# raynbowy23/RegT-GCN

Measured on AMD Instinct MI355X. Metric: training steps/sec (graph-snapshots/sec), higher is better.
Workload: dtype fp32; 1 GPU; cfg3: ONE synthetic regional graph, 100000 nodes / 1000000 edges / 8 regions, F=32, T=12, O=1, hidden=256; RegionalTemporalGCN forward+MSE+backward per snapshot, RMSprop step once per K steps (run.py semantics); gemm_arithmetic=fp32 MFMA (v_mfma_f32_32x32x2_f32), global_nodes=100000, global_edges=1000000, global_regions=8, parallelism=single GPU

## Files before the change

regt-gcn_amd/csrc/api.hip:

```cpp
#include <limits.h>
#include <stdarg.h>

#include <functional>
#include <initializer_list>
#include <map>
#include <mutex>
#include <string>
#include <unordered_map>
#include <vector>

#include "../../include/regtgcn.h"
#include <algorithm>
#include "kernels.h"

namespace regt {

static thread_local char g_err[512] = "";
void set_error(const char* fmt, ...) {
    va_list ap;
    va_start(ap, fmt);
    vsnprintf(g_err, sizeof(g_err), fmt, ap);
    va_end(ap);
}

// ... 707 lines not shown
    TRY(head_backward(d, p, gr, dpred, dhidden, hidden, L.y1, L.d1, L.dOH, L.kchunk_head, L.nchunks_head, rq, st));
    const bool split = gemm_mode() != 0 || !fp32_core_wide();
    if (split) {
        PROF("transpose_gate_w", st);
        TRY(launch_transpose3(p.gate_w[2] + C, p.gate_w[0] + C, p.gate_w[1] + C, 3, L.UT, C, C, 2L * C, st));
    }
    const bool wfr = abf && ibf && weights_frag(d) && d.regional;
    const WbPtrs wb = wb_ptrs(L.Wb, C, F, R);
    if (wfr) {
        CvtBatch cb{};
        cb.n = 3;
        for (int k = 0; k < 3; ++k) cb.t[k] = CvtTask{L.UT + (long)k * C * C, C, C, C, const_cast<float*>(wb.UT[k])};
        PROF("weights_bf16", st);
        TRY(launch_cvt_bf16_frag(cb, st));
    }
    const bool fused = wfr && !h_ext && fused_backward_ok(C) && fused_bwd_wanted();
    if (fused) {
        FusedBwdArgs a{};
        a.ZR = L.ZR; a.h = H; a.Ht = L.Ht; a.dOH = L.dOH; a.probs = L.probs;
        a.UhTf = wb.UT[0]; a.UzTf = wb.UT[1]; a.UrTf = wb.UT[2];
        a.dhp = L.dhp; a.dzr = L.dzr; a.dh = DH; a.rowdot = L.rowdot;
        a.M = M; a.T = T; a.slope = d.lrelu_slope; a.act_lrelu = d.regional ? 1 : 0; a.tile_ctr = L.tile_ctr;
        {
            PROF("fused_backward", st);
            TRY(launch_fused_backward(a, C, st));
        }
        if (gr.attention) {
            hipStream_t sa = side_fork(st);
            TRY(launch_rowdot_reduce(L.rowdot, L.dp_partial, N, T, L.cb_npb, sa));
            TRY(launch_att_bwd(L.dp_partial, L.cb_blocks, L.probs, gr.attention, T, sa));
        }
    } else {
    const bool gen = split && !ibf && !abf && gemm_dgrad1_gen_ok(M, C, N) && al16(L.Ht) && al16(L.dhp);
    if (gen) {
        GemmSegs S{};
        S.nseg = 1;
        S.seg[0] = make_seg(L.dhp, C, L.UT, nullptr, C, INT_MAX, C, true);
        S.row_div = T;
        EpiDgrad1 e{H, L.ZR, L.dOH, L.probs, L.dzr, DH, C, T};
        e.Ht = L.Ht; e.dhp = L.dhp; e.rowdot = L.rowdot; e.num_nodes = N;
        {
            PROF("dgrad_candidate", st);
            TRY(launch_gemm_dgrad1_gen(S, M, C, e, st));
        }
        if (gr.attention) {
            hipStream_t sa = side_fork(st);
            TRY(launch_rowdot_reduce(L.rowdot, L.dp_partial, N, T, L.cb_npb, sa, C / 128));
            TRY(launch_att_bwd(L.dp_partial, L.cb_blocks, L.probs, gr.attention, T, sa));
        }
    } else {
    {
        CellBwdArgs a{L.dOH, L.probs, L.ZR, H, L.Ht, L.dhp, L.dzr, L.dp_partial, N, T, C, L.cb_npb};
        a.out_bf16 = ibf; a.in_bf16 = abf;
        {
            PROF("cell_bwd", st);
            TRY(launch_cell_bwd(a, st));
        }
        if (gr.attention) TRY(launch_att_bwd(L.dp_partial, L.cb_blocks, L.probs, gr.attention, T, side_fork(st)));
    }
    {
        GemmSegs S{};
        S.nseg = 1;
        if (wfr) S.seg[0] = make_seg(L.dhp, C, wb.UT[0], nullptr, C, INT_MAX, C, true, SEG_A_BF16 | SEG_B_FRAG);
        else if (split) S.seg[0] = make_seg(L.dhp, C, L.UT, nullptr, C, INT_MAX, C, true, ibf ? SEG_A_BF16 : 0);
        else S.seg[0] = make_seg(L.dhp, C, p.gate_w[2] + C, nullptr, 2L * C, INT_MAX, C, false);
        S.row_div = T;
        EpiDgrad1 e{H, L.ZR, L.dOH, L.probs, L.dzr, DH, C, T};
        e.dzr_bf16 = ibf; e.h_bf16 = abf; e.zr_bf16 = abf; e.dh_bf16 = abf;
        PROF("dgrad_candidate", st);
        TRY(launch_gemm_dgrad1(S, M, C, e, st));
    }
    }
    if (!tcol) {
        GemmSegs S{};
        S.nseg = 2;
        if (wfr) {
            S.seg[0] = make_seg(byte_off(L.dzr, 2L * C), 2L * C, wb.UT[2], nullptr, C, INT_MAX, C, true, SEG_A_BF16 | SEG_B_FRAG);
            S.seg[1] = make_seg(L.dzr, 2L * C, wb.UT[1], nullptr, C, INT_MAX, C, true, SEG_A_BF16 | SEG_B_FRAG);
        } else if (split) {
            const int fl = ibf ? SEG_A_BF16 : 0;
            S.seg[0] = make_seg(byte_off(L.dzr, (ibf ? 2L : 4L) * C), 2L * C, L.UT + 2L * C * C, nullptr, C, INT_MAX, C, true, fl);
            S.seg[1] = make_seg(L.dzr, 2L * C, L.UT + (long)C * C, nullptr, C, INT_MAX, C, true, fl);
        } else {
            S.seg[0] = make_seg(L.dzr, 2L * C, p.gate_w[0] + C, nullptr, 2L * C, INT_MAX, C, false);
            S.seg[1] = make_seg(L.dzr + C, 2L * C, p.gate_w[1] + C, nullptr, 2L * C, INT_MAX, C, false);
        }
        S.row_div = T;
        EpiDgrad2 e{DH, H, C, d.regional ? ACT_LRELU : ACT_NONE, d.lrelu_slope};
        e.h_bf16 = abf; e.dh_bf16 = abf;
        PROF("dgrad_gates", st);
        TRY(launch_gemm_dgrad2(S, M, C, e, st));
    }
    }
    const int pairs_opt = option(OPT_WGRAD_PAIRS);
    const bool pairs = (pairs_opt == 2 ? wgrad_ring_active() : pairs_opt == 1) && ibf && qbf && abf && xbf && !h_ext && !tcol && C % 128 == 0 && F % 8 == 0;
    if (pairs) {
        int kc = L.kchunk, nc = L.nchunks;
        wgrad_ring_chunking(C, C + F, M, &kc, &nc);
        WgradArgs a{L.dhp, C, C, L.q, C, C + F, 0, M, kc, nullptr, nc, nullptr, 1};
        a.p_bf16 = 1; a.q_bf16 = 1; a.Q2 = L.AX; a.ldq2 = F; a.nin_split = C;
        TRY(rq.take((long)nc * wgrad_slab_stride(a), &a.slab));
        {
            PROF("wgrad_UhGh", st);
            TRY(launch_wgrad(a, st));
        }
        WgradReduceArgs r{};
        r.slab = a.slab; r.nchunks = nc; r.slab_stride = wgrad_slab_stride(a); r.slab_ld = C + F; r.ngroups = 1;
        r.elem_offset = 0; r.Nout = C; r.Nin = C; r.out = gr.gate_w[2] + C; r.ldo = 2L * C;
        r.colsum_out = L.dch; r.colsum_offset = (long)C * (C + F); r.ncolsum = C;
        TRY(rq.push(r));
        WgradReduceArgs g{};
        g.slab = a.slab; g.nchunks = nc; g.slab_stride = wgrad_slab_stride(a); g.slab_ld = C + F; g.ngroups = 1;
        g.elem_offset = C; g.Nout = C; g.Nin = F; g.out = L.dGh; g.ldo = F;
        TRY(rq.push(g));
    } else {
    {
        int kc = L.kchunk, nc = L.nchunks;
        if (!ibf && !qbf) wgrad_wide_chunking(C, C, M, &kc, &nc);
        TRY(wgrad_full(rq, "wgrad_Uh", L.dhp, C, C, L.q, C, C, 0, M, kc, nc, gr.gate_w[2] + C, 2L * C, L.dch, st, ibf, qbf));
    }
    {
        int kc = L.kchunk_s, nc = L.nchunks_s;
        if (!ibf && !xbf && F <= 32) wgrad_skinny_chunking(C, M, &kc, &nc);
        TRY(wgrad_full(rq, "wgrad_Gh", L.dhp, C, C, L.AX, F, F, 0, M, kc, nc, L.dGh, F, nullptr, st, ibf, xbf));
// ... 765 lines not shown
```

regt-gcn_amd/csrc/gemm.hip:

```cpp
#include "kernels.h"
#include "gemm_fast.h"
#include "gemm_split.h"
#include "gemm_small.h"

namespace regt {

#ifdef REGT_WG_TRACE
__device__ long g_wg_trace[4 * WG_TRACE_MAX];
__device__ long g_wg_marks[8 * WG_TRACE_MAX];
#define WG_TRACE_T(name) const long name = wall_clock64()
#define WG_TRACE_END(N, ta, tb)                                                                                              \
    if (threadIdx.x == 0 && WG_TILE_ID < WG_TRACE_MAX && (N) == REGT_WG_TRACE_N) {                                            \
        long* q_ = g_wg_trace + 4L * WG_TILE_ID;                                                                              \
        q_[0] = ta; q_[1] = tb; q_[2] = wall_clock64();                                                                       \
        q_[3] = ((long)__builtin_amdgcn_s_getreg((31 << 11) | 4)) | ((long)__builtin_amdgcn_s_getreg((31 << 11) | 20) << 32); \
    }
#else
#define WG_TRACE_T(name)
#define WG_TRACE_END(N, ta, tb)
#endif

__device__ __forceinline__ float fast_sigmoid(float x) { return __builtin_amdgcn_rcpf(1.0f + __expf(-x)); }
__device__ __forceinline__ float fast_tanh(float x) { return 1.0f - 2.0f * __builtin_amdgcn_rcpf(1.0f + __expf(2.0f * x)); }
__device__ __forceinline__ float4 ld4(const float* p) { return *reinterpret_cast<const float4*>(p); }
// ... 188 lines not shown
        if (V & 1) buf_st4_bf16(t.dzr, t.vdzr + i * t.sdzr, 0, REGT_V4(F_));
        else buf_st4(t.dzr, t.vdzr + i * t.sdzr, 0, REGT_V4(F_));
#undef F_
#define F_(k) cb_dh(v.k, a.R.k, a.p, a.d.k, a.Z.k)
        buf_st4(t.dh, t.vc + i * t.sc, 0, REGT_V4(F_));
#undef F_
    }
};
struct EpiDgrad1GenF {
    EpiDgrad1 e;
    int parts;
    static constexpr int ROUND_ROWS = 8;
    __device__ __forceinline__ static float half_wave_sum(float s) {
#define REGT_DPP_ADD(ctrl, rmask) s += __builtin_bit_cast(float, __builtin_amdgcn_update_dpp(0, __builtin_bit_cast(int, s), ctrl, rmask, 0xF, true))
        REGT_DPP_ADD(0xB1, 0xF);
        REGT_DPP_ADD(0x4E, 0xF);
        REGT_DPP_ADD(0x141, 0xF);
        REGT_DPP_ADD(0x140, 0xF);
        REGT_DPP_ADD(0x142, 0xA);
#undef REGT_DPP_ADD
        return s;
    }
    static constexpr int SUM_LANE = 31;
    static constexpr int EPI_AUX_BYTES = 192;
    struct Aux { float4 h, Z, R, d, t; float p; };
    __device__ __forceinline__ Aux load(long m, int c) const {
        const long node = m / e.T;
        Aux a;
        a.p = e.probs[(int)(m - node * e.T)];
        a.h = ld4(e.h + m * e.C + c);
        a.Z = ld4(e.ZR + m * (2L * e.C) + c);
        a.R = ld4(e.ZR + m * (2L * e.C) + e.C + c);
        a.d = ld4(e.dOH + node * e.C + c);
        a.t = ld4(e.Ht + m * e.C + c);
        return a;
    }
#define REGT_GEN_DOT(a) ((a.d.x * (a.Z.x * a.h.x + (1.0f - a.Z.x) * a.t.x) + a.d.y * (a.Z.y * a.h.y + (1.0f - a.Z.y) * a.t.y)) + \
                         (a.d.z * (a.Z.z * a.h.z + (1.0f - a.Z.z) * a.t.z) + a.d.w * (a.Z.w * a.h.w + (1.0f - a.Z.w) * a.t.w)))
    __device__ __forceinline__ void apply(long m, int c, float4 v, const Aux& a) const {
#define F_(k) cb_drp(v.k, a.h.k, a.R.k)
        st4(e.dzr + m * (2L * e.C) + e.C + c, REGT_V4(F_));
#undef F_
#define F_(k) cb_dh(v.k, a.R.k, a.p, a.d.k, a.Z.k)
        st4(e.dh + m * e.C + c, REGT_V4(F_));
#undef F_
#define F_(k) cb_dzp(__fmul_rn(a.p, a.d.k), a.h.k, a.t.k, a.Z.k)
        st4(e.dzr + m * (2L * e.C) + c, REGT_V4(F_));
#undef F_
        const float s = half_wave_sum(REGT_GEN_DOT(a));
        if ((threadIdx.x & 31) == SUM_LANE) e.rowdot[m * parts + c / GBN] = s;
    }
    static constexpr int NVAR = 1;
    static constexpr bool HAS_ROWTAB = true;
    struct Col {};
    struct Tile { __amdgpu_buffer_rsrc_t h, zr, d, dzr, dh, t, rd; int vc, vzr, sc, szr, vd, vrd, srd, rstep; const EpiRowEnt* rt; };
    __device__ __forceinline__ int variant(int) const { return 0; }
    __device__ __forceinline__ EpiRowEnt vrow(long m) const {
        const long node = m / e.T;
        return EpiRowEnt{(int)(node * e.C * 4), e.probs[(int)(m - node * e.T)]};
    }
    template <int V> __device__ __forceinline__ Col vcol(int) const { return Col{}; }
    template <int V> __device__ __forceinline__ Tile vtile(const EpiGeom& g) const {
        Tile t;
        t.h = buf_srd(e.h + g.m0 * e.C + g.n0);
        t.t = buf_srd(e.Ht + g.m0 * e.C + g.n0);
        t.dh = buf_srd(e.dh + g.m0 * e.C + g.n0);
        t.zr = buf_srd(e.ZR + g.m0 * (2L * e.C) + g.n0);
        t.d = buf_srd(e.dOH + g.n0);
        t.dzr = buf_srd(e.dzr + g.m0 * (2L * e.C) + g.n0);
        t.rd = buf_srd(e.rowdot + g.m0 * parts + g.n0 / GBN);
        t.vc = (g.rr * e.C + g.c) * 4;
        t.sc = g.step * e.C * 4;
        t.vzr = 2 * t.vc - g.c * 4;
        t.szr = 2 * t.sc;
        t.vd = g.c * 4;
        t.vrd = g.rr * parts * 4;
        t.srd = g.step * parts * 4;
        t.rt = g.rowtab + g.rr;
        t.rstep = g.step;
        return t;
    }
    struct VAux { float4 h, Z, R, d, t; float p; };
    template <int V> __device__ __forceinline__ VAux vload(const Tile& t, int i) const {
        const EpiRowEnt re = t.rt[i * t.rstep];
        VAux a;
        a.p = re.p;
        a.h = buf_ld4(t.h, t.vc, i * t.sc);
        a.Z = buf_ld4(t.zr, t.vzr, i * t.szr);
        a.R = buf_ld4(t.zr, t.vzr, i * t.szr + e.C * 4);
        a.d = buf_ld4(t.d, t.vd + re.off, 0);
        a.t = buf_ld4(t.t, t.vc, i * t.sc);
        return a;
    }
    template <int V> __device__ __forceinline__ void vapply(const Tile& t, int i, float4 v, const Col&, const VAux& a) const {
#define F_(k) cb_drp(v.k, a.h.k, a.R.k)
        buf_st4(t.dzr, t.vzr + i * t.szr + e.C * 4, 0, REGT_V4(F_));
#undef F_
#define F_(k) cb_dh(v.k, a.R.k, a.p, a.d.k, a.Z.k)
        buf_st4(t.dh, t.vc + i * t.sc, 0, REGT_V4(F_));
#undef F_
#define F_(k) cb_dzp(__fmul_rn(a.p, a.d.k), a.h.k, a.t.k, a.Z.k)
        buf_st4(t.dzr, t.vzr + i * t.szr, 0, REGT_V4(F_));
#undef F_
        const float s = half_wave_sum(REGT_GEN_DOT(a));
        if ((threadIdx.x & 31) == SUM_LANE) __builtin_amdgcn_raw_buffer_store_b32(__float_as_uint(s), t.rd, t.vrd + i * t.srd, 0, 0);
    }
#undef REGT_GEN_DOT
};
struct EpiDgrad2F {
    EpiDgrad2 e;
    __device__ __forceinline__ void operator()(long m, int c, float v) const {
        long i = m * e.C + c;
        float d = e.dh[i] + v;
        if (e.act == ACT_LRELU) d = e.h[i] > 0.f ? d : d * e.slope;
        e.dh[i] = d;
    }
    static constexpr int ROUND_ROWS = 16;
    struct Aux { float4 d, h; };
    __device__ __forceinline__ Aux load(long m, int c) const {
        Aux a;
        a.d = ld4(e.dh + m * e.C + c);
        a.h = e.act == ACT_LRELU ? ld4(e.h + m * e.C + c) : make_float4(1, 1, 1, 1);
        return a;
    }
    __device__ __forceinline__ void apply(long m, int c, float4 v, const Aux& a) const {
#define F_(k) ((a.d.k + v.k) * (a.h.k > 0.f ? 1.0f : e.slope))
        st4(e.dh + m * e.C + c, REGT_V4(F_));
#undef F_
    }
    static constexpr int NVAR = 2;
    static constexpr bool HAS_ROWTAB = false;
    struct Col {};
    struct VAux { float4 d, h; };
    struct Tile { __amdgpu_buffer_rsrc_t dh, h; int v, s; };
    __device__ __forceinline__ int variant(int) const { return e.act == ACT_LRELU ? 1 : 0; }
    template <int V> __device__ __forceinline__ Col vcol(int) const { return Col{}; }
    template <int V> __device__ __forceinline__ Tile vtile(const EpiGeom& g) const {
        Tile t;
        t.dh = buf_srd(e.dh + g.m0 * e.C + g.n0);
        if (V & 1) t.h = buf_srd(e.h + g.m0 * e.C + g.n0);
        t.v = (g.rr * e.C + g.c) * 4;
        t.s = g.step * e.C * 4;
        return t;
    }
    template <int V> __device__ __forceinline__ VAux vload(const Tile& t, int i) const {
        VAux a;
        a.d = buf_ld4(t.dh, t.v, i * t.s);
        if (V & 1) a.h = buf_ld4(t.h, t.v, i * t.s);
        return a;
    }
    template <int V> __device__ __forceinline__ void vapply(const Tile& t, int i, float4 v, const Col&, const VAux& a) const {
#define F_(k) ((a.d.k + v.k) * ((V & 1) ? (a.h.k > 0.f ? 1.0f : e.slope) : 1.0f))
        buf_st4(t.dh, t.v + i * t.s, 0, REGT_V4(F_));
#undef F_
    }
};
struct EpiMaskAddF {
    EpiMaskAdd e;
    __device__ __forceinline__ void operator()(long m, int c, float v) const {
        float o = e.mask[m * e.ldm + c] > 0.f ? v : 0.f;
        if (e.add) o += e.add[m * e.ldadd + c];
        e.out[m * e.ldo + c] = o;
    }
    static constexpr int ROUND_ROWS = 16;
    struct Aux { float4 mk, ad; };
    __device__ __forceinline__ Aux load(long m, int c) const {
        Aux a;
        a.mk = ld4(e.mask + m * e.ldm + c);
        a.ad = e.add ? ld4(e.add + m * e.ldadd + c) : make_float4(0, 0, 0, 0);
        return a;
    }
    __device__ __forceinline__ void apply(long m, int c, float4 v, const Aux& a) const {
#define F_(k) ((a.mk.k > 0.f ? v.k : 0.f) + a.ad.k)
        st4(e.out + m * e.ldo + c, REGT_V4(F_));
#undef F_
    }
    static constexpr int NVAR = 2;
    static constexpr bool HAS_ROWTAB = false;
    struct Col {};
    struct VAux { float4 mk, ad; };
    struct Tile { __amdgpu_buffer_rsrc_t out, mask, add; int vo, vm, va, so, sm, sa; };
    __device__ __forceinline__ int variant(int) const {
        return (e.ldo >= (1L << 22) || e.ldm >= (1L << 22) || (e.add && e.ldadd >= (1L << 22))) ? -1 : (e.add ? 1 : 0);
    }
    template <int V> __device__ __forceinline__ Col vcol(int) const { return Col{}; }
    template <int V> __device__ __forceinline__ Tile vtile(const EpiGeom& g) const {
        Tile t;
// ... 350 lines not shown
#pragma unroll
    for (int i = 0; i < 2; ++i)
#pragma unroll
        for (int j = 0; j < 2; ++j)
#pragma unroll
            for (int r = 0; r < 16; ++r) acc[i][j][r] = 0.f;
    WG_TRACE_T(t_a);
    if (uni) core.run_uniform(acc, relu_a != 0);
    else core.run(acc, relu_a != 0);
    WG_TRACE_T(t_b);
    core.for_each_vec_halves(acc, epi);
    WG_TRACE_END(N, t_a, t_b);
}

template <int NP>
__global__ __launch_bounds__(256, 2) void gemm_dgrad1_gen_kernel(GemmSegs S, long M, int N, EpiDgrad1GenF epi) {
    extern __shared__ __attribute__((aligned(16))) float lds[];
    const int tiles_n = (N + GBN - 1) / GBN;
    const int bid = xcd_remap(blockIdx.x, gridDim.x);
    const long m0 = (long)(bid / tiles_n) * GBM;
    const int n0 = (bid % tiles_n) * GBN;
    RowMap rm{m0, 1, (int)((M - m0) < GBM ? (M - m0) : GBM)};
    SplitCore<false, NP> core(S, rm, n0, N, lds, true);
    core.fill_rowtab(epi);
    f32x16 acc[2][2];
#pragma unroll
    for (int i = 0; i < 2; ++i)
#pragma unroll
        for (int j = 0; j < 2; ++j)
#pragma unroll
            for (int r = 0; r < 16; ++r) acc[i][j][r] = 0.f;
    const typename SplitCore<false, NP>::AGen g{epi.e.ZR, epi.e.Ht, epi.e.dOH, epi.e.dhp, epi.e.C, (unsigned)epi.e.num_nodes * (unsigned)epi.e.C * 4u};
    core.run_u_gen(acc, g);
    core.for_each_vec_halves(acc, epi);
}

template <class EpiF8, bool REGION>
__global__ __launch_bounds__(256, 3) void gemm_flat_split8_kernel(GemmSegs S, long M, int N, EpiF8 epi, int uniform) {
    extern __shared__ __attribute__((aligned(16))) float lds[];
    const int tiles_n = (N + GBN - 1) / GBN;
    const int bid = xcd_remap(blockIdx.x, gridDim.x);
    const long m0 = (long)(bid / tiles_n) * GBM;
    const int n0 = (bid % tiles_n) * GBN;
    RowMap rm{m0, 1, (int)((M - m0) < GBM ? (M - m0) : GBM)};
    SplitCore<REGION, 1> core(S, rm, n0, N, lds, true);
    core.fill_rowtab(epi);
    const bool uni = uniform != 0;
    if (!uni) core.plan();
    f32x16 acc[2][2];
#pragma unroll
    for (int i = 0; i < 2; ++i)
#pragma unroll
        for (int j = 0; j < 2; ++j)
#pragma unroll
            for (int r = 0; r < 16; ++r) acc[i][j][r] = 0.f;
    WG_TRACE_T(t_a);
    if (uniform == 2) core.run_uniform_frag(acc, false);
    else if (uni) core.run_uniform(acc, false);
    else core.run(acc, false);
    WG_TRACE_T(t_b);
    core.for_each_vec8_halves(acc, epi);
    WG_TRACE_END(N, t_a, t_b);
}

template <class EpiF, bool BT, bool REGION>
__global__ __launch_bounds__(256, 4) void gemm_flat_small_kernel(GemmSegs S, long M, int N, EpiF epi, int relu_a) {
// ... 173 lines not shown
    return launch_flat(S, M, N, EpiDgrad1F{e}, vec, st);
}
static bool dgrad1_gen_wanted() { return option(OPT_DGRAD1_GEN) != 0; }
bool gemm_dgrad1_gen_ok(long M, int C, int num_nodes) {
    return dgrad1_gen_wanted() && (gemm_mode() == 0 || gemm_mode() == 1) && !fp32_core_wide() && !gemm_desc_table_forced() && C % GBN == 0 && C % GBK == 0 &&
           (long)cdiv(M, GBM) * (C / GBN) >= SMALL_TILE_LIMIT && M < (1L << 31) && (long)num_nodes * C * 4 < (1L << 31) &&
           (long)C * 8 * (GBM + 1) < (1L << 31);
}
int launch_gemm_dgrad1_gen(const GemmSegs& S, long M, int N, const EpiDgrad1& e, hipStream_t st) {
    REGT_CHECK_ARG(N == e.C && S.nseg == 1 && S.seg[0].K == e.C && (S.seg[0].flags & SEG_BT) && (S.seg[0].flags & SEG_VEC_B) &&
                   !(S.seg[0].flags & (SEG_A_BF16 | SEG_B_FRAG | SEG_REGION | SEG_REPEAT)), "dgrad1 (generated operand): one [N][K] weight segment with K = C");
    REGT_CHECK_ARG(gemm_dgrad1_gen_ok(M, e.C, e.num_nodes), "dgrad1 (generated operand): shape / arithmetic not covered");
    REGT_CHECK_ARG(e.Ht && e.dhp && e.rowdot && !e.dzr_bf16 && !e.h_bf16 && !e.zr_bf16 && !e.dh_bf16, "dgrad1 (generated operand): fp32 arrays, all outputs given");
    REGT_CHECK_ARG(a16(e.h) && a16(e.ZR) && a16(e.dOH) && a16(e.dzr) && a16(e.dh) && a16(e.Ht) && a16(e.dhp), "dgrad1 (generated operand): 16-byte aligned arrays");
    const long tiles = (long)cdiv(M, GBM) * (N / GBN);
    REGT_CHECK_ARG(tiles < (1L << 31), "gemm: too many tiles");
    if (gemm_mode() == 1)
        hipLaunchKernelGGL(gemm_dgrad1_gen_kernel<3>, dim3((unsigned)tiles), dim3(256), SplitGeom<3>::LDS_BYTES, st, S, M, N, EpiDgrad1GenF{e, e.C / GBN});
    else
        hipLaunchKernelGGL(gemm_dgrad1_gen_kernel<0>, dim3((unsigned)tiles), dim3(256), SplitGeom<0>::LDS_BYTES, st, S, M, N, EpiDgrad1GenF{e, e.C / GBN});
    REGT_CHECK_LAUNCH();
    return REGT_OK;
}
int launch_gemm_dgrad2(const GemmSegs& S, long M, int N, const EpiDgrad2& e, hipStream_t st) {
    REGT_CHECK_ARG(N == e.C, "dgrad2 gemm expects N == C");
    const bool vec = e.C % 4 == 0 && a16(e.dh) && a16(e.h);
    if (e.h_bf16 || e.dh_bf16) {
        REGT_CHECK_ARG(fast_class(S, N, vec) == 1 && e.C % 8 == 0, "dgrad2 gemm: bf16-stored activations need the bf16-operand vector path");
        return launch_split8<EpiDgrad28F, false>(S, M, N, EpiDgrad28F{e}, st);
    }
    if (fast_class(S, N, vec) == 1) return launch_fast<EpiDgrad2F, true, false>(S, M, N, EpiDgrad2F{e}, 0, st);
    if (fast_class(S, N, vec) == 0) return launch_fast<EpiDgrad2F, false, false>(S, M, N, EpiDgrad2F{e}, 0, st);
    return launch_flat(S, M, N, EpiDgrad2F{e}, vec, st);
}
int launch_gemm_mask_add(const GemmSegs& S, long M, int N, const EpiMaskAdd& e, hipStream_t st) {
    const bool vec = N % 4 == 0 && e.ldo % 4 == 0 && e.ldm % 4 == 0 && (!e.add || e.ldadd % 4 == 0) && a16(e.out) &&
                     a16(e.mask) && a16(e.add);
    if (fast_class(S, N, vec) == 0) return launch_fast<EpiMaskAddF, false, false>(S, M, N, EpiMaskAddF{e}, 0, st);
    return launch_flat(S, M, N, EpiMaskAddF{e}, vec, st);
}

__global__ __launch_bounds__(256, 1) void gemm_cand_kernel(CandArgs a) {
    extern __shared__ __attribute__((aligned(16))) float lds[];
    const int tiles_n = (a.C + GBN - 1) / GBN;
    const long C = a.C;
    f32x16 acc[2][2];
    const int bid = xcd_remap(blockIdx.x, gridDim.x);
    const int i0 = (bid / tiles_n) * GBM;
    const int n0 = (bid % tiles_n) * GBN;
    const int nvalid = (a.num_nodes - i0) < GBM ? (a.num_nodes - i0) : GBM;
    f32x16 oh[2][2];
#pragma unroll
    for (int i = 0; i < 2; ++i)
#pragma unroll
        for (int j = 0; j < 2; ++j)
#pragma unroll
            for (int r = 0; r < 16; ++r) oh[i][j][r] = 0.f;
    for (int t = 0; t < a.T; ++t) {
        RowMap rm{(long)i0 * a.T + t, a.T, nvalid};
        GemmCore core(a.S, rm, n0, a.C, lds);
#pragma unroll
        for (int i = 0; i < 2; ++i)
#pragma unroll
            for (int j = 0; j < 2; ++j)
#pragma unroll
                for (int r = 0; r < 16; ++r) acc[i][j][r] = 0.f;
// ... 635 lines not shown
```

regt-gcn_amd/csrc/gemm_split.h:

```cpp
#pragma once
#include <type_traits>
#include "gemm_fast.h"

namespace regt {

typedef __bf16 bf16x8 __attribute__((ext_vector_type(8)));
typedef __bf16 bf16x2 __attribute__((ext_vector_type(2)));
typedef float f32x2 __attribute__((ext_vector_type(2)));

constexpr int SP_ROW_B = 32;
constexpr int SP_PLANE_B = 128 * SP_ROW_B;
constexpr int CP_ROW_B = 64;
__device__ __forceinline__ constexpr int cp_off(int r, int g) { return r * CP_ROW_B + ((g ^ ((r >> 2) & 3)) << 4); }
template <int NP>
struct SplitGeom {
    static constexpr int OPER_B = NP == 0 ? 128 * CP_ROW_B : NP * SP_PLANE_B;
    static constexpr int STAGE_B = 2 * OPER_B;
    static constexpr int EPI_HALF_B = 64 * G_LDS_KROW * 4;
    static constexpr int TABLE_OFF_B = 2 * STAGE_B > EPI_HALF_B ? 2 * STAGE_B : EPI_HALF_B;
    static constexpr int LDS_BYTES = TABLE_OFF_B + G_TABLE_BYTES;
    static_assert(2 * STAGE_B <= 2 * G_STAGE * 4, "split stages fit the fp32 core's LDS footprint (table offset, epilogue image)");
};
constexpr int SP_LDS_BYTES = SplitGeom<3>::LDS_BYTES;
__device__ __forceinline__ constexpr int sp_off(int r, int g) { return r * SP_ROW_B + ((g ^ ((r >> 3) & 1)) << 4); }
// ... 208 lines not shown
        store_half<RELU>(1, ra, rb, held);
        {
            const bool two = nslab > 1;
            if (two) cursor_next(c);
            const SrdsU d = make_u(c, two);
            load_half(0, d, ra, rb);
            load_half(1, d, ra, rb);
            held = d.abf;
        }
        __syncthreads();
        compute(0, acc);
        for (int it = 0; it + 1 < nslab; ++it) {
            const bool live = it + 2 < nslab;
            if (live) cursor_next(c);
            const SrdsU nx = make_u(c, live);
            __syncthreads();
            fused<RELU>(0, 1, nx, ra, rb, acc, held);
            __syncthreads();
            fused<RELU>(1, 0, nx, ra, rb, acc, held);
            held = nx.abf;
        }
        __syncthreads();
        compute(1, acc);
        __syncthreads();
    }

    struct AGen {
        const float* ZR; const float* Ht; const float* dOH; float* dhp;
        int C; unsigned doh_bytes;
    };
    struct GenRegs { float4 z[4], t[4], d[4]; };
    struct GenRows { int vz[2], vh[2], vd[2]; float p[2]; };
    struct GenSrd { __amdgpu_buffer_rsrc_t z, t, d, o; };
    __device__ __forceinline__ GenRows gen_rows(const AGen& g) const {
        GenRows r;
#pragma unroll
        for (int j = 0; j < 2; ++j) {
            const int rl = (tid >> 2) + 64 * j;
            const EpiRowEnt re = Base::rowtab()[rl];
            r.p[j] = re.p;
            r.vd[j] = re.off + (tid & 3) * 16;
            r.vz[j] = rl * g.C * 8 + (tid & 3) * 16;
            r.vh[j] = rl * g.C * 4 + (tid & 3) * 16;
        }
        return r;
    }
    __device__ __forceinline__ GenSrd gen_srd(const AGen& g, bool live, bool writer) const {
        GenSrd s;
        const int C = g.C;
        s.z = __builtin_amdgcn_make_buffer_rsrc(const_cast<float*>(g.ZR + rm.base * 2L * C), 0, live ? rm.nvalid * C * 8 : 0, 0x00020000);
        s.t = __builtin_amdgcn_make_buffer_rsrc(const_cast<float*>(g.Ht + rm.base * (long)C), 0, live ? rm.nvalid * C * 4 : 0, 0x00020000);
        s.d = __builtin_amdgcn_make_buffer_rsrc(const_cast<float*>(g.dOH), 0, live ? (int)g.doh_bytes : 0, 0x00020000);
        s.o = __builtin_amdgcn_make_buffer_rsrc(g.dhp + rm.base * (long)C, 0, writer ? rm.nvalid * C * 4 : 0, 0x00020000);
        return s;
    }
    __device__ __forceinline__ void gen_load_half(int h, const GenSrd& s, const GenRows& r, int k0, GenRegs& q) const {
        const int so = (k0 + 16 * h) * 4;
#pragma unroll
        for (int j = 0; j < 2; ++j) {
            q.z[h + 2 * j] = buf_ld4(s.z, r.vz[j], so);
            q.t[h + 2 * j] = buf_ld4(s.t, r.vh[j], so);
            q.d[h + 2 * j] = buf_ld4(s.d, r.vd[j], so);
        }
    }
    __device__ __forceinline__ void gen_store_half(int h, const GenSrd& s, const GenRows& r, int k0, const GenRegs& q, const float4 (&rb)[4]) const {
        char* st = reinterpret_cast<char*>(lds) + h * STAGE_B;
        const int ko = (k0 + 16 * h) * 4;
#pragma unroll
        for (int j = 0; j < 2; ++j) {
            const int off = cp_off((tid >> 2) + 64 * j, tid & 3);
            const float4 z = q.z[h + 2 * j], t = q.t[h + 2 * j], d = q.d[h + 2 * j];
            const float p = r.p[j];
            float4 a;
            a.x = cb_dhp(__fmul_rn(p, d.x), z.x, t.x); a.y = cb_dhp(__fmul_rn(p, d.y), z.y, t.y);
            a.z = cb_dhp(__fmul_rn(p, d.z), z.z, t.z); a.w = cb_dhp(__fmul_rn(p, d.w), z.w, t.w);
            if constexpr (NP == 0) {
                *reinterpret_cast<float4*>(st + off) = a;
                *reinterpret_cast<float4*>(st + OPER_B + off) = rb[h + 2 * j];
            } else {
// ... 59 lines not shown
        compute(1, acc);
        __syncthreads();
    }
    __device__ __forceinline__ void fused_gen(int hs, int hc, const SrdsU& nx, const GenSrd& sn, const GenSrd& sw, const GenRows& rows,
                                              int k_held, int k_next, GenRegs& q, float4 (&rb)[4], f32x16 (&acc)[2][2]) const {
        __builtin_amdgcn_sched_barrier(0);
        const Frags f = read_frags(hc);
        gen_store_half(hs, sw, rows, k_held, q, rb);
        mfmas(f, acc);
        gen_load_half(hs, sn, rows, k_next, q);
        load_b_half(hs, nx, rb);
        if constexpr (NP == 0) {
            __builtin_amdgcn_sched_group_barrier(0x100, 8, 0);
#pragma unroll
            for (int r = 0; r < 8; ++r) {
                __builtin_amdgcn_sched_group_barrier(0x008, 1, 0);
                __builtin_amdgcn_sched_group_barrier(0x006, 8, 0);
                if (r < 4) __builtin_amdgcn_sched_group_barrier(0x200, 1, 0);
                else __builtin_amdgcn_sched_group_barrier(0x020, 2, 0);
                if (r >= 2 && r < 4) __builtin_amdgcn_sched_group_barrier(0x040, 1, 0);
            }
        } else {
            __builtin_amdgcn_sched_group_barrier(0x100, 12, 0);
#pragma unroll
            for (int r = 0; r < 24; ++r) {
                __builtin_amdgcn_sched_group_barrier(0x008, 1, 0);
                __builtin_amdgcn_sched_group_barrier(0x002, 5, 0);
                if (r & 1) __builtin_amdgcn_sched_group_barrier(0x200, 1, 0);
                if (r >= 16) __builtin_amdgcn_sched_group_barrier(0x020, 1, 0);
                if (r >= 6 && r < 8) __builtin_amdgcn_sched_group_barrier(0x040, 1, 0);
            }
        }
        __builtin_amdgcn_sched_barrier(0);
    }

    struct FragsB { bf16x8 a[2][NP ? NP : 1], b[2][NP ? NP : 1]; };
    struct FragsF { float4 a[2][2], b[2][2]; };
    using Frags = std::conditional_t<NP == 0, FragsF, FragsB>;
    __device__ __forceinline__ Frags read_frags(int h) const {
        const char* st = reinterpret_cast<const char*>(lds) + h * STAGE_B;
        const int lr = lane & 31, lh = lane >> 5;
        Frags f;
        if constexpr (NP == 0) {
#pragma unroll
            for (int kk = 0; kk < 2; ++kk)
#pragma unroll
                for (int t = 0; t < 2; ++t) {
                    f.a[t][kk] = *reinterpret_cast<const float4*>(st + cp_off(wr * 64 + t * 32 + lr, 2 * kk + lh));
                    f.b[t][kk] = *reinterpret_cast<const float4*>(st + OPER_B + cp_off(wc * 64 + t * 32 + lr, 2 * kk + lh));
                }
            return f;
        } else {
#pragma unroll
        for (int p = NP - 1; p >= 0; --p)
#pragma unroll
            for (int t = 0; t < 2; ++t) {
                f.a[t][p] = *reinterpret_cast<const bf16x8*>(st + p * SP_PLANE_B + sp_off(wr * 64 + t * 32 + lr, lh));
                f.b[t][NP - 1 - p] = *reinterpret_cast<const bf16x8*>(st + OPER_B + (NP - 1 - p) * SP_PLANE_B + sp_off(wc * 64 + t * 32 + lr, lh));
            }
        return f;
        }
    }
    static constexpr int NPROD = NP == 3 ? 6 : 1;
    __device__ __forceinline__ static void mfmas(const Frags& f, f32x16 (&acc)[2][2]) {
        if constexpr (NP == 0) {
#pragma unroll
// ... 557 lines not shown
```

regt-gcn_amd/csrc/kernels.h:

```cpp
#pragma once
#include "gemm_core.h"
#include "options.h"

namespace regt {
#ifdef REGT_WG_TRACE
#ifndef REGT_WG_TRACE_N
#define REGT_WG_TRACE_N 512
#endif
constexpr int WG_TRACE_MAX = 40000;
extern __device__ long g_wg_marks[8 * WG_TRACE_MAX];
#define WG_TILE_ID ((int)(rm.base / 128) * ((N + 127) / 128) + n0 / 128)
#define WG_MARK(i) do { if (threadIdx.x == 0 && WG_TILE_ID < WG_TRACE_MAX && N == REGT_WG_TRACE_N) g_wg_marks[8L * WG_TILE_ID + (i)] = wall_clock64(); } while (0)
#else
#define WG_MARK(i) do { } while (0)
#endif

typedef unsigned int u32x4_t __attribute__((ext_vector_type(4)));
typedef unsigned int u32x2_t __attribute__((ext_vector_type(2)));
__device__ __forceinline__ __amdgpu_buffer_rsrc_t buf_srd(const void* p) {
    const unsigned long long a = reinterpret_cast<unsigned long long>(p);
    const unsigned lo = __builtin_amdgcn_readfirstlane((unsigned)a);
    const unsigned hi = __builtin_amdgcn_readfirstlane((unsigned)(a >> 32));
    return __builtin_amdgcn_make_buffer_rsrc(reinterpret_cast<void*>(((unsigned long long)hi << 32) | lo), 0, 0x7FFFFFF0, 0x00020000);
}
// ... 13 lines not shown
                       __builtin_bit_cast(unsigned, __builtin_convertvector(hi, bf16x2_t))};
    __builtin_amdgcn_raw_buffer_store_b64(w, r, voff, soff, 0);
}
__device__ __forceinline__ float gru_blend(float Z, float h, float ht) { return fmaf(Z, h, __fmul_rn(1.0f - Z, ht)); }
__device__ __forceinline__ float cb_dhp(float g, float z, float ht) { return __fmul_rn(__fmul_rn(g, 1.0f - z), fmaf(-ht, ht, 1.0f)); }
__device__ __forceinline__ float cb_dzp(float g, float h, float ht, float z) { return __fmul_rn(__fmul_rn(g, h - ht), __fmul_rn(z, 1.0f - z)); }
__device__ __forceinline__ float cb_drp(float dq, float h, float r) { return __fmul_rn(__fmul_rn(dq, h), __fmul_rn(r, 1.0f - r)); }
__device__ __forceinline__ float cb_dh(float dq, float r, float p, float d, float z) { return fmaf(dq, r, __fmul_rn(__fmul_rn(p, d), z)); }
__device__ __forceinline__ float cb_ds(float dh, float acc, float factor) { return __fmul_rn(dh + acc, factor); }

struct EpiRowEnt { int off; float p; };
struct EpiGeom { long m0; int n0, rr, c, step; const EpiRowEnt* rowtab; };
constexpr int EPI_ROWTAB_BYTES = 128 * (int)sizeof(EpiRowEnt);


enum : int { ACT_NONE = 0, ACT_LRELU = 1, ACT_RELU = 2, ACT_SIGMOID = 3, ACT_TANH = 4 };

struct EpiBiasAct {
    float* out; long ldo; const float* bias; int act; float slope;
    int out_bf16 = 0;
};
struct EpiGates {
    float* ZR;
    const float* h; float* q; const float* bias; int C;
    int q_bf16 = 0;
    int h_bf16 = 0, zr_bf16 = 0;
};
struct EpiDgrad1 {
    const float* h; const float* ZR; const float* dOH; const float* probs;
    float* dzr; float* dh; int C; int T;
    int dzr_bf16 = 0;
    int h_bf16 = 0, zr_bf16 = 0, dh_bf16 = 0;
    const float* Ht = nullptr; float* dhp = nullptr; float* rowdot = nullptr; int num_nodes = 0;
};
struct EpiDgrad2 {
    float* dh; const float* h; int C; int act; float slope;
    int h_bf16 = 0, dh_bf16 = 0;
};
struct EpiMaskAdd {
    float* out; long ldo; const float* mask; long ldm; const float* add; long ldadd;
};

int launch_gemm_bias_act(const GemmSegs& S, long M, int N, const EpiBiasAct& e, hipStream_t st);
int launch_gemm_gates(const GemmSegs& S, long M, int N, const EpiGates& e, hipStream_t st);
int launch_gemm_dgrad1(const GemmSegs& S, long M, int N, const EpiDgrad1& e, hipStream_t st);
bool gemm_dgrad1_gen_ok(long M, int C, int num_nodes);
bool wgrad_ring_chunking(int Nout, int Nin, long M, int* kchunk, int* nchunks);
bool wgrad_skinny_chunking(int Nout, long M, int* kchunk, int* nchunks);
bool wgrad_wide_chunking(int Nout, int Nin, long M, int* kchunk, int* nchunks);
long wgrad_chunk_bound(int Nout, int Nin, long M);
bool wgrad_ring_active();
int launch_gemm_dgrad1_gen(const GemmSegs& S, long M, int N, const EpiDgrad1& e, hipStream_t st);
int launch_gemm_dgrad2(const GemmSegs& S, long M, int N, const EpiDgrad2& e, hipStream_t st);
int launch_gemm_mask_add(const GemmSegs& S, long M, int N, const EpiMaskAdd& e, hipStream_t st);

struct CandArgs {
    GemmSegs S;
    int num_nodes, T, C;
    const float* bias;
    const float* ZR;
    const float* h;
    const float* probs;
    float* Ht;
    float* OH;
    int act_bf16 = 0;
    int node_sum_rows = 64;
};
int launch_gemm_candidate(const CandArgs& a, hipStream_t st);

struct WgradArgs {
    const float* P; long ldp; int Nout;
    const float* Q; long ldq; int Nin;
    int q_relu;
    long M;
    int kchunk;
    const int* chunk_tab;
    int nchunks;
    float* slab;
    int colsum;
    const float* Q2 = nullptr; long ldq2 = 0; int nin_split = 0;
    int p_bf16 = 0, q_bf16 = 0;
    int all_csum = 0;
};
int launch_wgrad(const WgradArgs& a, hipStream_t st);
long wgrad_slab_stride(const WgradArgs& a);

// ... 193 lines not shown
```

Before: 64.48 snapshots/s.

## Generate dz operand inside dgrad-gates GEMM instead of materializing it in dgrad1

When the generated-operand dgrad path is taken, dgrad1 runs in a lean variant that skips loading Ht and skips writing the dz half of dzr and the rowdot partials. The dgrad-gates GEMM instead recomputes dz on the fly from ZR, Ht, h and dOH as its A operand. The tile owning column zero writes dzr and per-row dot sums for the attention backward. This is meant to remove one materialize-then-reread of the dz tensor and move the Ht traffic into the second GEMM. The cost is more register pressure and more loads per slab in the new kernel, and the attention reduce now waits until after dgrad2.

Result: slower. 56.99 snapshots/s (-11.6%).

```diff
diff --git a/regt-gcn_amd/csrc/api.hip b/regt-gcn_amd/csrc/api.hip
--- a/regt-gcn_amd/csrc/api.hip
+++ b/regt-gcn_amd/csrc/api.hip
@@ -763,18 +763,19 @@
         }
     } else {
     const bool gen = split && !ibf && !abf && gemm_dgrad1_gen_ok(M, C, N) && al16(L.Ht) && al16(L.dhp);
+    const bool bal = gen && !tcol && !h_ext;
     if (gen) {
         GemmSegs S{};
         S.nseg = 1;
         S.seg[0] = make_seg(L.dhp, C, L.UT, nullptr, C, INT_MAX, C, true);
         S.row_div = T;
         EpiDgrad1 e{H, L.ZR, L.dOH, L.probs, L.dzr, DH, C, T};
-        e.Ht = L.Ht; e.dhp = L.dhp; e.rowdot = L.rowdot; e.num_nodes = N;
+        e.Ht = L.Ht; e.dhp = L.dhp; e.rowdot = L.rowdot; e.num_nodes = N; e.lean = bal ? 1 : 0;
         {
             PROF("dgrad_candidate", st);
             TRY(launch_gemm_dgrad1_gen(S, M, C, e, st));
         }
-        if (gr.attention) {
+        if (gr.attention && !bal) {
             hipStream_t sa = side_fork(st);
             TRY(launch_rowdot_reduce(L.rowdot, L.dp_partial, N, T, L.cb_npb, sa, C / 128));
             TRY(launch_att_bwd(L.dp_partial, L.cb_blocks, L.probs, gr.attention, T, sa));
@@ -819,8 +820,21 @@
         S.row_div = T;
         EpiDgrad2 e{DH, H, C, d.regional ? ACT_LRELU : ACT_NONE, d.lrelu_slope};
         e.h_bf16 = abf; e.dh_bf16 = abf;
-        PROF("dgrad_gates", st);
-        TRY(launch_gemm_dgrad2(S, M, C, e, st));
+        if (bal) {
+            e.ZR = L.ZR; e.Ht = L.Ht; e.dOH = L.dOH; e.probs = L.probs; e.dzr = L.dzr; e.rowdot = L.rowdot; e.T = T; e.num_nodes = N;
+            {
+                PROF("dgrad_gates", st);
+                TRY(launch_gemm_dgrad2_gen(S, M, C, e, st));
+            }
+            if (gr.attention) {
+                hipStream_t sa = side_fork(st);
+                TRY(launch_rowdot_reduce(L.rowdot, L.dp_partial, N, T, L.cb_npb, sa, 1));
+                TRY(launch_att_bwd(L.dp_partial, L.cb_blocks, L.probs, gr.attention, T, sa));
+            }
+        } else {
+            PROF("dgrad_gates", st);
+            TRY(launch_gemm_dgrad2(S, M, C, e, st));
+        }
     }
     }
     const int pairs_opt = option(OPT_WGRAD_PAIRS);
diff --git a/regt-gcn_amd/csrc/gemm.hip b/regt-gcn_amd/csrc/gemm.hip
--- a/regt-gcn_amd/csrc/gemm.hip
+++ b/regt-gcn_amd/csrc/gemm.hip
@@ -244,7 +244,7 @@
         a.Z = ld4(e.ZR + m * (2L * e.C) + c);
         a.R = ld4(e.ZR + m * (2L * e.C) + e.C + c);
         a.d = ld4(e.dOH + node * e.C + c);
-        a.t = ld4(e.Ht + m * e.C + c);
+        a.t = e.lean ? make_float4(0, 0, 0, 0) : ld4(e.Ht + m * e.C + c);
         return a;
     }
 #define REGT_GEN_DOT(a) ((a.d.x * (a.Z.x * a.h.x + (1.0f - a.Z.x) * a.t.x) + a.d.y * (a.Z.y * a.h.y + (1.0f - a.Z.y) * a.t.y)) + \
@@ -256,17 +256,18 @@
 #define F_(k) cb_dh(v.k, a.R.k, a.p, a.d.k, a.Z.k)
         st4(e.dh + m * e.C + c, REGT_V4(F_));
 #undef F_
+        if (e.lean) return;
 #define F_(k) cb_dzp(__fmul_rn(a.p, a.d.k), a.h.k, a.t.k, a.Z.k)
         st4(e.dzr + m * (2L * e.C) + c, REGT_V4(F_));
 #undef F_
         const float s = half_wave_sum(REGT_GEN_DOT(a));
         if ((threadIdx.x & 31) == SUM_LANE) e.rowdot[m * parts + c / GBN] = s;
     }
-    static constexpr int NVAR = 1;
+    static constexpr int NVAR = 2;
     static constexpr bool HAS_ROWTAB = true;
     struct Col {};
     struct Tile { __amdgpu_buffer_rsrc_t h, zr, d, dzr, dh, t, rd; int vc, vzr, sc, szr, vd, vrd, srd, rstep; const EpiRowEnt* rt; };
-    __device__ __forceinline__ int variant(int) const { return 0; }
+    __device__ __forceinline__ int variant(int) const { return e.lean ? 1 : 0; }
     __device__ __forceinline__ EpiRowEnt vrow(long m) const {
         const long node = m / e.T;
         return EpiRowEnt{(int)(node * e.C * 4), e.probs[(int)(m - node * e.T)]};
@@ -275,12 +276,12 @@
     template <int V> __device__ __forceinline__ Tile vtile(const EpiGeom& g) const {
         Tile t;
         t.h = buf_srd(e.h + g.m0 * e.C + g.n0);
-        t.t = buf_srd(e.Ht + g.m0 * e.C + g.n0);
+        if (!(V & 1)) t.t = buf_srd(e.Ht + g.m0 * e.C + g.n0);
         t.dh = buf_srd(e.dh + g.m0 * e.C + g.n0);
         t.zr = buf_srd(e.ZR + g.m0 * (2L * e.C) + g.n0);
         t.d = buf_srd(e.dOH + g.n0);
         t.dzr = buf_srd(e.dzr + g.m0 * (2L * e.C) + g.n0);
-        t.rd = buf_srd(e.rowdot + g.m0 * parts + g.n0 / GBN);
+        if (!(V & 1)) t.rd = buf_srd(e.rowdot + g.m0 * parts + g.n0 / GBN);
         t.vc = (g.rr * e.C + g.c) * 4;
         t.sc = g.step * e.C * 4;
         t.vzr = 2 * t.vc - g.c * 4;
@@ -301,7 +302,7 @@
         a.Z = buf_ld4(t.zr, t.vzr, i * t.szr);
         a.R = buf_ld4(t.zr, t.vzr, i * t.szr + e.C * 4);
         a.d = buf_ld4(t.d, t.vd + re.off, 0);
-        a.t = buf_ld4(t.t, t.vc, i * t.sc);
+        if (!(V & 1)) a.t = buf_ld4(t.t, t.vc, i * t.sc);
         return a;
     }
     template <int V> __device__ __forceinline__ void vapply(const Tile& t, int i, float4 v, const Col&, const VAux& a) const {
@@ -311,6 +312,7 @@
 #define F_(k) cb_dh(v.k, a.R.k, a.p, a.d.k, a.Z.k)
         buf_st4(t.dh, t.vc + i * t.sc, 0, REGT_V4(F_));
 #undef F_
+        if (V & 1) return;
 #define F_(k) cb_dzp(__fmul_rn(a.p, a.d.k), a.h.k, a.t.k, a.Z.k)
         buf_st4(t.dzr, t.vzr + i * t.szr, 0, REGT_V4(F_));
 #undef F_
@@ -365,6 +367,13 @@
 #define F_(k) ((a.d.k + v.k) * ((V & 1) ? (a.h.k > 0.f ? 1.0f : e.slope) : 1.0f))
         buf_st4(t.dh, t.v + i * t.s, 0, REGT_V4(F_));
 #undef F_
+    }
+};
+struct EpiDgrad2GenF : EpiDgrad2F {
+    static constexpr bool HAS_ROWTAB = true;
+    __device__ __forceinline__ EpiRowEnt vrow(long m) const {
+        const long node = m / e.T;
+        return EpiRowEnt{(int)(node * e.C * 4), e.probs[(int)(m - node * e.T)]};
     }
 };
 struct EpiMaskAddF {
@@ -781,6 +790,29 @@
             for (int r = 0; r < 16; ++r) acc[i][j][r] = 0.f;
     const typename SplitCore<false, NP>::AGen g{epi.e.ZR, epi.e.Ht, epi.e.dOH, epi.e.dhp, epi.e.C, (unsigned)epi.e.num_nodes * (unsigned)epi.e.C * 4u};
     core.run_u_gen(acc, g);
+    core.for_each_vec_halves(acc, epi);
+}
+
+template <int NP>
+__global__ __launch_bounds__(256, 2) void gemm_dgrad2_gen_kernel(GemmSegs S, long M, int N, EpiDgrad2GenF epi) {
+    extern __shared__ __attribute__((aligned(16))) float lds[];
+    const int tiles_n = (N + GBN - 1) / GBN;
+    const int bid = xcd_remap(blockIdx.x, gridDim.x);
+    const long m0 = (long)(bid / tiles_n) * GBM;
+    const int n0 = (bid % tiles_n) * GBN;
+    RowMap rm{m0, 1, (int)((M - m0) < GBM ? (M - m0) : GBM)};
+    SplitCore<false, NP> core(S, rm, n0, N, lds, true);
+    core.fill_rowtab(epi);
+    f32x16 acc[2][2];
+#pragma unroll
+    for (int i = 0; i < 2; ++i)
+#pragma unroll
+        for (int j = 0; j < 2; ++j)
+#pragma unroll
+            for (int r = 0; r < 16; ++r) acc[i][j][r] = 0.f;
+    const typename SplitCore<false, NP>::ZGen g{epi.e.ZR, epi.e.Ht, epi.e.h, epi.e.dOH, epi.e.dzr, epi.e.rowdot, epi.e.C,
+                                                (unsigned)epi.e.num_nodes * (unsigned)epi.e.C * 4u};
+    core.run_u_gen2(acc, g);
     core.for_each_vec_halves(acc, epi);
 }
 
@@ -1020,6 +1052,23 @@
     if (fast_class(S, N, vec) == 1) return launch_fast<EpiDgrad2F, true, false>(S, M, N, EpiDgrad2F{e}, 0, st);
     if (fast_class(S, N, vec) == 0) return launch_fast<EpiDgrad2F, false, false>(S, M, N, EpiDgrad2F{e}, 0, st);
     return launch_flat(S, M, N, EpiDgrad2F{e}, vec, st);
+}
+int launch_gemm_dgrad2_gen(const GemmSegs& S, long M, int N, const EpiDgrad2& e, hipStream_t st) {
+    REGT_CHECK_ARG(N == e.C && S.nseg == 2, "dgrad2 (generated operand): two segments, N == C");
+    for (int q = 0; q < 2; ++q)
+        REGT_CHECK_ARG(S.seg[q].K == e.C && (S.seg[q].flags & SEG_BT) && (S.seg[q].flags & SEG_VEC_B) &&
+                       !(S.seg[q].flags & (SEG_A_BF16 | SEG_B_FRAG | SEG_REGION | SEG_REPEAT | SEG_RELU_A)), "dgrad2 (generated operand): [N][K] weight segments with K = C");
+    REGT_CHECK_ARG(gemm_dgrad1_gen_ok(M, e.C, e.num_nodes) && uniform_ok(S, M) == 1 && e.C >= 2 * GBK, "dgrad2 (generated operand): shape / arithmetic not covered");
+    REGT_CHECK_ARG(e.ZR && e.Ht && e.dOH && e.probs && e.dzr && e.rowdot && e.T > 0 && !e.h_bf16 && !e.dh_bf16, "dgrad2 (generated operand): fp32 arrays, all given");
+    REGT_CHECK_ARG(a16(e.h) && a16(e.ZR) && a16(e.dOH) && a16(e.dzr) && a16(e.dh) && a16(e.Ht) && a16(S.seg[0].A), "dgrad2 (generated operand): 16-byte aligned arrays");
+    const long tiles = (long)cdiv(M, GBM) * (N / GBN);
+    REGT_CHECK_ARG(tiles < (1L << 31), "gemm: too many tiles");
+    if (gemm_mode() == 1)
+        hipLaunchKernelGGL(gemm_dgrad2_gen_kernel<3>, dim3((unsigned)tiles), dim3(256), SplitGeom<3>::LDS_BYTES, st, S, M, N, EpiDgrad2GenF{{e}});
+    else
+        hipLaunchKernelGGL(gemm_dgrad2_gen_kernel<0>, dim3((unsigned)tiles), dim3(256), SplitGeom<0>::LDS_BYTES, st, S, M, N, EpiDgrad2GenF{{e}});
+    REGT_CHECK_LAUNCH();
+    return REGT_OK;
 }
 int launch_gemm_mask_add(const GemmSegs& S, long M, int N, const EpiMaskAdd& e, hipStream_t st) {
     const bool vec = N % 4 == 0 && e.ldo % 4 == 0 && e.ldm % 4 == 0 && (!e.add || e.ldadd % 4 == 0) && a16(e.out) &&
diff --git a/regt-gcn_amd/csrc/gemm_split.h b/regt-gcn_amd/csrc/gemm_split.h
--- a/regt-gcn_amd/csrc/gemm_split.h
+++ b/regt-gcn_amd/csrc/gemm_split.h
@@ -264,7 +264,7 @@
     struct GenRegs { float4 z[4], t[4], d[4]; };
     struct GenRows { int vz[2], vh[2], vd[2]; float p[2]; };
     struct GenSrd { __amdgpu_buffer_rsrc_t z, t, d, o; };
-    __device__ __forceinline__ GenRows gen_rows(const AGen& g) const {
+    __device__ __forceinline__ GenRows gen_rows_c(int C) const {
         GenRows r;
 #pragma unroll
         for (int j = 0; j < 2; ++j) {
@@ -272,11 +272,12 @@
             const EpiRowEnt re = Base::rowtab()[rl];
             r.p[j] = re.p;
             r.vd[j] = re.off + (tid & 3) * 16;
-            r.vz[j] = rl * g.C * 8 + (tid & 3) * 16;
-            r.vh[j] = rl * g.C * 4 + (tid & 3) * 16;
+            r.vz[j] = rl * C * 8 + (tid & 3) * 16;
+            r.vh[j] = rl * C * 4 + (tid & 3) * 16;
         }
         return r;
     }
+    __device__ __forceinline__ GenRows gen_rows(const AGen& g) const { return gen_rows_c(g.C); }
     __device__ __forceinline__ GenSrd gen_srd(const AGen& g, bool live, bool writer) const {
         GenSrd s;
         const int C = g.C;
@@ -402,6 +403,157 @@
             }
         }
         __builtin_amdgcn_sched_barrier(0);
+    }
+
+    struct ZGen {
+        const float* ZR; const float* Ht; const float* h; const float* dOH; float* dzr; float* rowdot;
+        int C; unsigned doh_bytes;
+    };
+    struct ZRegs { float4 z[4], t[4], h[4], d[4]; };
+    struct ZSrd { __amdgpu_buffer_rsrc_t z, t, h, d; };
+    __device__ __forceinline__ ZSrd zgen_srd(const ZGen& g, bool live) const {
+        ZSrd s;
+        const int C = g.C;
+        s.z = __builtin_amdgcn_make_buffer_rsrc(const_cast<float*>(g.ZR + rm.base * 2L * C), 0, live ? rm.nvalid * C * 8 : 0, 0x00020000);
+        s.t = __builtin_amdgcn_make_buffer_rsrc(const_cast<float*>(g.Ht + rm.base * (long)C), 0, live ? rm.nvalid * C * 4 : 0, 0x00020000);
+        s.h = __builtin_amdgcn_make_buffer_rsrc(const_cast<float*>(g.h + rm.base * (long)C), 0, live ? rm.nvalid * C * 4 : 0, 0x00020000);
+        s.d = __builtin_amdgcn_make_buffer_rsrc(const_cast<float*>(g.dOH), 0, live ? (int)g.doh_bytes : 0, 0x00020000);
+        return s;
+    }
+    __device__ __forceinline__ void zgen_load_half(int h, const ZSrd& s, const GenRows& r, int k0, ZRegs& q) const {
+        const int so = (k0 + 16 * h) * 4;
+#pragma unroll
+        for (int j = 0; j < 2; ++j) {
+            q.z[h + 2 * j] = buf_ld4(s.z, r.vz[j], so);
+            q.t[h + 2 * j] = buf_ld4(s.t, r.vh[j], so);
+            q.h[h + 2 * j] = buf_ld4(s.h, r.vh[j], so);
+            q.d[h + 2 * j] = buf_ld4(s.d, r.vd[j], so);
+        }
+    }
+    template <bool W>
+    __device__ __forceinline__ void zgen_store_half(int h, __amdgpu_buffer_rsrc_t o, const GenRows& r, int k0, const ZRegs& q,
+                                                    const float4 (&rb)[4], float (&dot)[2]) const {
+        char* st = reinterpret_cast<char*>(lds) + h * STAGE_B;
+        const int ko = (k0 + 16 * h) * 4;
+#pragma unroll
+        for (int j = 0; j < 2; ++j) {
+            const int off = cp_off((tid >> 2) + 64 * j, tid & 3);
+            const float4 z = q.z[h + 2 * j], t = q.t[h + 2 * j], hh = q.h[h + 2 * j], d = q.d[h + 2 * j];
+            const float p = r.p[j];
+            float4 a;
+            a.x = cb_dzp(__fmul_rn(p, d.x), hh.x, t.x, z.x); a.y = cb_dzp(__fmul_rn(p, d.y), hh.y, t.y, z.y);
+            a.z = cb_dzp(__fmul_rn(p, d.z), hh.z, t.z, z.z); a.w = cb_dzp(__fmul_rn(p, d.w), hh.w, t.w, z.w);
+            if constexpr (NP == 0) {
+                *reinterpret_cast<float4*>(st + off) = a;
+                *reinterpret_cast<float4*>(st + OPER_B + off) = rb[h + 2 * j];
+            } else {
+                const int offs = sp_off((tid >> 2) + 64 * j, (tid >> 1) & 1) + (tid & 1) * 8;
+                asm volatile("" : "+v"(a.x), "+v"(a.y), "+v"(a.z), "+v"(a.w));
+                split_store(st + offs, a);
+                split_store(st + OPER_B + offs, rb[h + 2 * j]);
+            }
+            if constexpr (W) {
+                buf_st4(o, r.vz[j] + ko, 0, a);
+                dot[j] += (d.x * (z.x * hh.x + (1.0f - z.x) * t.x) + d.y * (z.y * hh.y + (1.0f - z.y) * t.y)) +
+                          (d.z * (z.z * hh.z + (1.0f - z.z) * t.z) + d.w * (z.w * hh.w + (1.0f - z.w) * t.w));
+            }
+        }
+    }
+    template <bool HG, bool NG, bool W>
+    __device__ __forceinline__ void fused_z(int hs, int hc, const SrdsU& nx, const ZSrd& sn, __amdgpu_buffer_rsrc_t o, const GenRows& rows,
+                                            int k_held, int k_next, ZRegs& q, float4 (&rb)[4], float (&dot)[2], f32x16 (&acc)[2][2]) const {
+        __builtin_amdgcn_sched_barrier(0);
+        const Frags f = read_frags(hc);
+        if constexpr (HG) zgen_store_half<W>(hs, o, rows, k_held, q, rb, dot);
+        else store_half<false>(hs, q.z, rb);
+        mfmas(f, acc);
+        if constexpr (NG) {
+            zgen_load_half(hs, sn, rows, k_next, q);
+            load_b_half(hs, nx, rb);
+        } else {
+            load_half(hs, nx, q.z, rb);
+        }
+        if constexpr (NP == 0) {
+            __builtin_amdgcn_sched_group_barrier(0x100, 8, 0);
+#pragma unroll
+            for (int r = 0; r < (HG ? 12 : 8); ++r) {
+                __builtin_amdgcn_sched_group_barrier(0x008, 1, 0);
+                if (r < 8) __builtin_amdgcn_sched_group_barrier(0x006, HG ? (W ? 12 : 8) : 6, 0);
+                if (r < 4) __builtin_amdgcn_sched_group_barrier(0x200, 1, 0);
+                else if (r >= (HG ? 8 : 4)) __builtin_amdgcn_sched_group_barrier(0x020, NG ? 3 : 1, 0);
+                if (HG && W && r >= 2 && r < 4) __builtin_amdgcn_sched_group_barrier(0x040, 1, 0);
+            }
+        } else {
+            __builtin_amdgcn_sched_group_barrier(0x100, 12, 0);
+#pragma unroll
+            for (int r = 0; r < 24; ++r) {
+                __builtin_amdgcn_sched_group_barrier(0x008, 1, 0);
+                __builtin_amdgcn_sched_group_barrier(0x002, HG ? (W ? 7 : 5) : 4, 0);
+                if (r & 1) __builtin_amdgcn_sched_group_barrier(0x200, 1, 0);
+                if (r >= (HG ? 19 : 16)) __builtin_amdgcn_sched_group_barrier(0x020, NG ? 2 : 1, 0);
+                if (HG && W && r >= 6 && r < 8) __builtin_amdgcn_sched_group_barrier(0x040, 1, 0);
+            }
+        }
+        __builtin_amdgcn_sched_barrier(0);
+    }
+    __device__ __forceinline__ void run_u_gen2(f32x16 (&acc)[2][2], const ZGen& g) {
+        static_assert(NP == 0 || NP == 3, "generated A operand: fp32 storage (fp32 MFMA or the exact bf16x3 split)");
+        nreg_u = 0;
+        const int nA = S.seg[0].K / GBK, nslab = nA + S.seg[1].K / GBK;
+        const bool writer = n0 == 0;
+        auto cur = [&](int i) { return i < nA ? SegCursor{0, 0, i * GBK} : SegCursor{1, 0, (i - nA) * GBK}; };
+        __syncthreads();
+        const GenRows rows = gen_rows_c(g.C);
+        ZRegs q;
+        float4 rb[4];
+        float dot[2] = {0.f, 0.f};
+        {
+            const SrdsU d = make_u(cur(0), true);
+            load_half(0, d, q.z, rb);
+            load_half(1, d, q.z, rb);
+            store_half<false>(0, q.z, rb);
+            store_half<false>(1, q.z, rb);
+        }
+        {
+            const SrdsU d = make_u(cur(1), true);
+            load_half(0, d, q.z, rb);
+            load_half(1, d, q.z, rb);
+        }
+        __syncthreads();
+        compute(0, acc);
+        const __amdgpu_buffer_rsrc_t so = __builtin_amdgcn_make_buffer_rsrc(g.dzr + rm.base * 2L * g.C, 0, writer ? rm.nvalid * g.C * 8 : 0, 0x00020000);
+        int k_held = GBK;
+        for (int it = 0; it + 1 < nslab; ++it) {
+            const bool live = it + 2 < nslab;
+            const bool hg = it + 1 >= nA, ng = live ? it + 2 >= nA : hg;
+            const SegCursor c = cur(live ? it + 2 : 0);
+            const SrdsU nx = make_u(c, live);
+            const ZSrd sn = zgen_srd(g, live && ng);
+            const int k_next = c.k0;
+#define REGT_Z_STEP(hs)                                                                                                        \
+    __syncthreads();                                                                                                           \
+    if (!hg && !ng) fused_z<false, false, false>(hs, 1 - hs, nx, sn, so, rows, k_held, k_next, q, rb, dot, acc);               \
+    else if (!hg) fused_z<false, true, false>(hs, 1 - hs, nx, sn, so, rows, k_held, k_next, q, rb, dot, acc);                  \
+    else if (writer) fused_z<true, true, true>(hs, 1 - hs, nx, sn, so, rows, k_held, k_next, q, rb, dot, acc);                 \
+    else fused_z<true, true, false>(hs, 1 - hs, nx, sn, so, rows, k_held, k_next, q, rb, dot, acc);
+            REGT_Z_STEP(0)
+            REGT_Z_STEP(1)
+#undef REGT_Z_STEP
+            k_held = k_next;
+        }
+        __syncthreads();
+        compute(1, acc);
+        if (writer) {
+#pragma unroll
+            for (int j = 0; j < 2; ++j) {
+                float s = dot[j];
+                s += __builtin_bit_cast(float, __builtin_amdgcn_update_dpp(0, __builtin_bit_cast(int, s), 0xB1, 0xF, 0xF, true));
+                s += __builtin_bit_cast(float, __builtin_amdgcn_update_dpp(0, __builtin_bit_cast(int, s), 0x4E, 0xF, 0xF, true));
+                const int rl = (tid >> 2) + 64 * j;
+                if ((tid & 3) == 0 && rl < rm.nvalid) g.rowdot[rm.base + rl] = s;
+            }
+        }
+        __syncthreads();
     }
 
     struct FragsB { bf16x8 a[2][NP ? NP : 1], b[2][NP ? NP : 1]; };
diff --git a/regt-gcn_amd/csrc/kernels.h b/regt-gcn_amd/csrc/kernels.h
--- a/regt-gcn_amd/csrc/kernels.h
+++ b/regt-gcn_amd/csrc/kernels.h
@@ -69,10 +69,13 @@
     int dzr_bf16 = 0;
     int h_bf16 = 0, zr_bf16 = 0, dh_bf16 = 0;
     const float* Ht = nullptr; float* dhp = nullptr; float* rowdot = nullptr; int num_nodes = 0;
+    int lean = 0;
 };
 struct EpiDgrad2 {
     float* dh; const float* h; int C; int act; float slope;
     int h_bf16 = 0, dh_bf16 = 0;
+    const float* ZR = nullptr; const float* Ht = nullptr; const float* dOH = nullptr; const float* probs = nullptr;
+    float* dzr = nullptr; float* rowdot = nullptr; int T = 0, num_nodes = 0;
 };
 struct EpiMaskAdd {
     float* out; long ldo; const float* mask; long ldm; const float* add; long ldadd;
@@ -89,6 +92,7 @@
 bool wgrad_ring_active();
 int launch_gemm_dgrad1_gen(const GemmSegs& S, long M, int N, const EpiDgrad1& e, hipStream_t st);
 int launch_gemm_dgrad2(const GemmSegs& S, long M, int N, const EpiDgrad2& e, hipStream_t st);
+int launch_gemm_dgrad2_gen(const GemmSegs& S, long M, int N, const EpiDgrad2& e, hipStream_t st);
 int launch_gemm_mask_add(const GemmSegs& S, long M, int N, const EpiMaskAdd& e, hipStream_t st);
 
 struct CandArgs {
```
